# google/uis-rnn

Measured on NVIDIA H100. Metric: predict_frames_per_sec_beam10_256d, higher is better.
Workload: dtype f32

## Files before the change

### uisrnn_b200/csrc/uis_beam.cuh

```cuda
#pragma once
#include "uis_common.cuh"
#include "uis_beam_tc.cuh"
#include "uis_beam_stat.cuh"

namespace uis {

constexpr int kStages = 2;
constexpr int kStageBytes = 48 * 1024;
constexpr int kInitSlot = 0;
#ifndef UIS_CP_BEAM
#define UIS_CP_BEAM 20
#endif
constexpr int kCPBeam = UIS_CP_BEAM;
template <int H> struct BeamCP { static constexpr int value = H > 512 ? 8 : kCPBeam; };
template <int H> __host__ __device__ constexpr int beam_cp() { return BeamCP<H>::value; }
constexpr int kCPCluster = 12;
constexpr int kXchVals = 24;
constexpr int kCPTree = 16;
template <int H> struct TreeCP { static constexpr int value = H > 512 ? 8 : kCPTree; };
template <int H> __host__ __device__ constexpr int tree_cp() { return TreeCP<H>::value; }
constexpr int kMaxLanes = 8;
constexpr int kMaxBeam = 128;
constexpr int kMaxDepth = 4;

// ... 37 lines not shown
  alignas(64) CUtensorMap tc_wmap;
  float tc_sh, tc_sa;
  float tc_inv_hh, tc_inv_1, tc_inv_2;
  float* tc_scratch;
  SmemLayout tc_layout;
  unsigned* stat_bar;
  float* stat_scratch;
  float* pool_mean;
  float* pool_hidden;
  float* pool_mse;
  unsigned* bp;
  int* queue;
  int* labels;
  int* status;
  unsigned long long* stats;
  int trace_utt;
  int trace_capacity;
  int* dbg_win;
  float* dbg_score;
  long long* dbg_off;
  float* dbg_final_scores;
  int* dbg_final_k;
  float* dbg_best_mean;
  float* dbg_best_hidden;
  int* dbg_best_blocks;
  unsigned char* tree_arena;
  int tree_spill_all;
};

template <int V> struct Pow2Floor { static constexpr int value = (V >= 2) ? 2 * Pow2Floor<V / 2>::value : 1; };
template <> struct Pow2Floor<1> { static constexpr int value = 1; };
template <> struct Pow2Floor<0> { static constexpr int value = 1; };
constexpr int cmin(int a, int b) { return a < b ? a : b; }

template <int H_, int D_, int CP_ = kCPBeam>
struct Cfg {
  static constexpr int H = H_, D = D_;
  static constexpr int CP = CP_;
  static constexpr int UPT = (H >= 512) ? 2 : 1;
  static constexpr int NT = H / UPT;
  static constexpr int NW = NT / 32;
  static constexpr bool REBALANCE = (NT == 256);
  static constexpr int PRODUCER_THREADS = REBALANCE ? 128 : 32;
  static constexpr int BLOCK = NT + PRODUCER_THREADS;
  static constexpr int RG = 3 * UPT;
  static constexpr int KG1 = UPT, TG1 = NT / KG1, R1 = H / TG1;
  static constexpr int R2 = (UPT == 2) ? 4 : 1, KG2 = NT * R2 / D, TG2 = NT / KG2;
  static constexpr int KT_HH = Pow2Floor<kStageBytes / (12 * H)>::value;
  static constexpr int KT_1 = cmin(Pow2Floor<kStageBytes / (4 * H)>::value, H);
  static constexpr int KT_2 = cmin(Pow2Floor<kStageBytes / (4 * D)>::value, H);
  static constexpr int N_HH = H / KT_HH, N_1 = H / KT_1, N_2 = H / KT_2;
  static constexpr int TILES_PER_PASS = N_HH + N_1 + N_2;
  static_assert(H % KT_HH == 0 && H % KT_1 == 0 && H % KT_2 == 0, "tile split");
  static_assert(KT_1 % KG1 == 0 && KT_2 % KG2 == 0, "K split");
  static_assert(TG2 * R2 == D && TG1 * R1 == H, "row split");
  static_assert(KG1 * H <= 2 * H && KG2 * D <= 2 * H, "K-split scratch must fit in XA+XB");
  static_assert(D % 4 == 0 && NT % 32 == 0 && D <= NT, "shape");
};

__host__ __device__ inline unsigned align_up(unsigned v, unsigned a) { return (v + a - 1) / a * a; }

enum { LS_U = 0, LS_N, LS_TN, LS_T, LS_NB, LS_GEN, LS_ACTIVE, LS_FAILED, LS_TRACED, LS_NFINITE, LS_KMAX,
       LS_NWIN, LS_ERR, LS_M, LS_COLBASE, LS_NE, LS_ROW0_LO, LS_ROW0_HI, LS_DBGROWS_LO, LS_DBGROWS_HI,
       LS_FRESH, LS_COUNT = 24 };
enum { MI_PUBLISHED = 0, MI_DONE, MI_MTOT, MI_QNEXT, MI_NLIST, MI_MAXK };

template <int H, int D, int kCP = kCPBeam, bool XCL = false, int TCN = 0, bool STAT = false>
__host__ __device__ inline SmemLayout make_layout(int B, int Kcap, int G) {
  SmemLayout L;
  unsigned o = 0;
  if constexpr (TCN > 0) {
    using TC = TcCfg<H, D, TCN>;
    L.ring = o;  o += TC::STAGES * kTcBoxBytes;
    L.xa = o;    o += TC::BOP_BYTES;
    L.xb = o;
  } else {
    L.ring = o;  o += STAT ? align_up(StatCfg<H, D>::BYTES, 128) : kStages * kStageBytes;
    L.xa = o;    o += H * kCP * 4;
    L.xb = o;    o += H * kCP * 4;
  }
  L.wv = o;    o += D * 4;
  unsigned q = 0;
  L.l_xt = q;      q += 2 * D * 4;
  L.l_tabs = q;    q += 2u * B * Kcap * 16;
  L.l_meta = q;    q += 2u * 4 * B * 4;
  L.l_candoff = q; q += align_up((B + 1) * 4, 16);
  const unsigned ne = (unsigned)B * (Kcap + 1);
  L.l_keys = q;    q += align_up(ne * 8, 16);
  L.l_svals = q;   q += align_up(ne * 4, 16);
  L.l_wins = q;    q += align_up(3u * B * 4, 16);
  L.l_wcol = q;    q += align_up((unsigned)B * 4, 16);
  L.l_lcol = q;    q += align_up(2u * B * 4, 16);
  const unsigned pw = ((unsigned)B * Kcap + B + 1 + 31) / 32;
  L.l_used = q;    q += align_up(pw * 4, 16);
  L.l_scored = q;  q += align_up(pw * 4, 16);
  L.l_ls = q;      q += LS_COUNT * 4;
  L.lane_stride = align_up(q, 16);
  L.lanes = o;     o += L.lane_stride * G;
// ... 465 lines not shown
    const int m = i / H, k = i % H;
    XA[(size_t)k * CP + m] = __ldcg(pool_hidden_g + (size_t)cc.lane[m0 + m] * lane_pool_h + (size_t)cc.dst[m0 + m] * H + k);
  }
  named_bar_sync(1, NT);
  stat_dot<H, S::R1, CP, NT>(sW, S::LD, S::R0, XA, XB, Mp, tid);
  named_bar_sync(1, NT);
  if (tid < S::R1 * CP) {
    const int m = tid % CP, u = tid / CP, j = q * S::R1 + u;
    if (m < Mp)
      scratch_g[(size_t)m * H + j] = fmaxf(__fadd_rn(stat_sum<S::R1, CP, NT>(XB, u, m), __ldg(p.b1 + j)), 0.f);
  }
  stat_group_sync<NT>(bar, epoch, tid);
  if (tid == 0) { const long long now_ = clock64(); ph[3] += now_ - tmark; tmark = now_; }
  for (int i = tid; i < Mp * H; i += NT) {
    const int m = i / H, k = i % H;
    XA[(size_t)k * CP + m] = __ldcg(scratch_g + (size_t)m * H + k);
  }
  named_bar_sync(1, NT);
  stat_dot<H, S::R2, CP, NT>(sW, S::LD, S::R0 + S::R1, XA, XB, Mp, tid);
  named_bar_sync(1, NT);
  if (tid < S::R2 * CP) {
    const int m = tid % CP, u = tid / CP, d = q * S::R2 + u;
    if (m < Mp) {
      const float mval = __fadd_rn(stat_sum<S::R2, CP, NT>(XB, u, m), __ldg(p.b2 + d));
      const int n = cc.vis[m0 + m];
      const float mu_old = __ldcg(pool_mean_g + (size_t)cc.lane[m0 + m] * lane_pool_m + (size_t)cc.src[m0 + m] * D + d);
      const float mu = (n == 0) ? mval : __fdiv_rn(__fadd_rn(__fmul_rn(mu_old, (float)(n - 1)), mval), (float)n);
      pool_mean_g[(size_t)cc.lane[m0 + m] * lane_pool_m + (size_t)cc.dst[m0 + m] * D + d] = mu;
    }
  }
  stat_group_sync<NT>(bar, epoch, tid);
}

template <int H, int D, int N, class Idle>
__device__ __forceinline__ void tc_run_pass(const BeamParams& p, const unsigned char* ring, unsigned char* bop,
                                            const TcBars& tb, unsigned& tbox, const ColCtx cc, int m0, int Mp,
                                            float* pool_mean_cta, float* pool_hidden_cta, float* scratch_cta, int tid,
                                            int lane, int warp, long long* ph, long long& tmark, long long* tstat,
                                            Idle idle_work) {
  using TC = TcCfg<H, D, N>;
  constexpr int NT = 256, NI = N / 8;
  constexpr int KB = (NI == 6) ? 2 : 4, WB = (NI == 6) ? 3 : NI;
  auto hslot = [&](int g, int s) { return pool_hidden_cta + (size_t)(g * p.P + s) * H; };
  auto mslot = [&](int g, int s) { return pool_mean_cta + (size_t)(g * p.P + s) * D; };
  const int wg = warp >> 2;
  const int r0 = wg * 64 + (warp & 3) * 16 + (lane >> 2);
  const int cq = 2 * (lane & 3);
  long long* ts = (tid == 0) ? tstat : nullptr;
  const long long t_in = clock64();
  float acc[TC::NACC];
  auto stage_b = [&](auto src, float scale) {
    const long long w0 = clock64();
    tc_gather_b<H, N, NT>(bop, src, Mp, scale, tid);
    tc_publish_b<NT>();
    if (ts) ts[2] += clock64() - w0;
  };
  if (tid < Mp && (tid == 0 || cc.lane[m0 + tid] != cc.lane[m0 + tid - 1]))
    prefetch_l2_bulk(p.gi + (size_t)cc.girow[m0 + tid] * 3 * H, 3 * H * 4);
  stage_b([&](int m) -> const float* {
    return hslot(cc.lane[m0 + m], cc.src[m0 + m]); }, p.tc_sh);
  if (tid == 0) { const long long now_ = clock64(); ph[1] += now_ - tmark; tmark = now_; }
  idle_work();
  if (tid == 0) { const long long now_ = clock64(); ph[7] += now_ - tmark; tmark = now_; }
  static_assert(H >= NT, "gate parking: 2 * (N / 2) * NT floats within the [N][H] scratch");
  float* park = scratch_cta + tid;
  for (int ut = 0; ut < TC::UT; ++ut) {
    const int j0 = ut * 128 + r0;
    {
      float v[TC::NV];
#pragma unroll
      for (int g = 0; g < 2; ++g) {
        tc_tile<TC>(acc, ring, bop, tb, tbox, wg, lane, ts);
        tc_fold<TC>(acc, v, p.tc_inv_hh);
        const float bh[2] = {__ldg(p.bhh + g * H + j0), __ldg(p.bhh + g * H + j0 + 8)};
#pragma unroll
        for (int q = 0; q < TC::NV; ++q) park[(g * TC::NV + q) * NT] = __fadd_rn(v[q], bh[(q >> 1) & 1]);
      }
    }
    tc_tile<TC>(acc, ring, bop, tb, tbox, wg, lane, ts);
    float an[TC::NV];
    tc_fold<TC>(acc, an, p.tc_inv_hh);
    {
      const float bh[2] = {__ldg(p.bhh + 2 * H + j0), __ldg(p.bhh + 2 * H + j0 + 8)};
#pragma unroll
      for (int q = 0; q < TC::NV; ++q) an[q] = __fadd_rn(an[q], bh[(q >> 1) & 1]);
    }
#pragma unroll
    for (int k0 = 0; k0 < 2 * NI; k0 += KB) {
      float gr[KB][2], gz[KB][2], gn[KB][2], pr[KB][2], pz[KB][2], ho[KB][2];
#pragma unroll
      for (int b = 0; b < KB; ++b) {
        const int i = (k0 + b) >> 1, e = (k0 + b) & 1, m = 8 * i + cq + e;
        if (m < Mp) {
          const float* gi = p.gi + (size_t)cc.girow[m0 + m] * 3 * H + j0;
          const float* hs = hslot(cc.lane[m0 + m], cc.src[m0 + m]) + j0;
#pragma unroll
// ... 109 lines not shown
  uint64_t* empty = full + (TC ? TCC::STAGES : kStages);
  volatile int* misc = reinterpret_cast<volatile int*>(smem + L.misc);
  TcBars tb{full, empty};

  const int tid = threadIdx.x, lane = tid & 31, warp = tid >> 5;

  if (tid == 0) {
    if constexpr (TC) {
      for (int s = 0; s < TCC::STAGES; ++s) {
        mbar_init(&tb.full[s], 1);
        mbar_init(&tb.empty[s], NW);
      }
    } else {
      for (int s = 0; s < kStages; ++s) {
        mbar_init(&full[s], 1);
        mbar_init(&empty[s], NW);
      }
    }
    for (int i = 0; i < 16; ++i) misc[i] = 0;
    if constexpr (TC)
      for (int i = 16; i < 20; ++i) reinterpret_cast<long long*>(smem + L.phase)[i] = 0;
    if constexpr (XCL) {
      uint64_t* xbar = reinterpret_cast<uint64_t*>(smem + L.xbar);
      mbar_init(&xbar[0], cluster_nctarank() - 1);
      mbar_init(&xbar[1], cluster_nctarank() - 1);
      misc[MI_QNEXT] = (int)cluster_id_x();
    }
    if constexpr (STAT) misc[MI_QNEXT] = sgroup;
    fence_mbar_init();
  }
  __syncthreads();
  if constexpr (XCL) cluster_sync_all();

  if (warp >= NW) {
    if constexpr (STAT) return;
    if constexpr (TC) asm volatile("setmaxnreg.dec.sync.aligned.u32 40;");
    else if constexpr (C::REBALANCE) asm volatile("setmaxnreg.dec.sync.aligned.u32 24;");
    if constexpr (TC) {
      if (warp == NW) tc_producer_loop<TCC, H>(&p.tc_wmap, reinterpret_cast<unsigned char*>(ring), tb, &misc[MI_DONE]);
    } else {
      if (warp == NW && lane == 0) producer_loop<C, XCL>(p, ring, full, empty, misc);
    }
    return;
  }
  if constexpr (TC) asm volatile("setmaxnreg.inc.sync.aligned.u32 232;");
  else if constexpr (C::REBALANCE && !STAT) asm volatile("setmaxnreg.inc.sync.aligned.u32 240;");

  auto lane_base = [&](int g) -> unsigned char* { return smem + L.lanes + (size_t)g * L.lane_stride; };
  auto LSp = [&](int g) -> volatile int* { return reinterpret_cast<volatile int*>(lane_base(g) + L.l_ls); };
  const int DH = p.depth * H;
  const size_t pool_m_stride = (size_t)p.P * D, pool_h_stride = (size_t)p.P * DH;
  float* pool_mean_cta = p.pool_mean + (size_t)(STAT ? sgroup : blockIdx.x) * G * pool_m_stride;
  float* pool_hidden_cta = p.pool_hidden + (size_t)(STAT ? sgroup : blockIdx.x) * G * pool_h_stride;
  unsigned* bp_cta = p.bp + (size_t)blockIdx.x * G * p.maxN * B;
  const unsigned PW = (unsigned)(p.P + 31) / 32;
  const float INF = __int_as_float(0x7f800000);
  const int bbits = B > 32 ? 7 : 5;

  float bh[C::RG], b1r[UPT];
#pragma unroll
  for (int i = 0; i < C::RG; ++i) bh[i] = TC ? 0.f : p.bhh[(i / UPT) * H + tid + NT * (i % UPT)];
#pragma unroll
  for (int u = 0; u < UPT; ++u) b1r[u] = TC ? 0.f : p.b1[tid + NT * u];
  const float b2r = (tid < D && !TC) ? p.b2[tid] : 0.f;
  unsigned tc_boxes = 0;
  float* tc_scratch_cta = TC ? p.tc_scratch + (size_t)blockIdx.x * (TC ? TCN : 1) * H : nullptr;
  if (tid < D) wv[tid] = p.wvec[tid];
  unsigned stat_epoch = 0;
  if constexpr (STAT) stat_load_weights<H, D, NT>(ring, p.whh_t, p.w1_t, p.w2_t, sq, tid);
  for (int g = 0; g < G; ++g) {
    if (tid < D) pool_mean_cta[g * pool_m_stride + (size_t)kInitSlot * D + tid] = p.mean0[tid];
    for (int q = tid; q < DH; q += NT) pool_hidden_cta[g * pool_h_stride + (size_t)kInitSlot * DH + q] = p.hidden0[q];
  }

  int* collane = colarr; int* colsrc = colarr + G * B; int* colnew = colarr + 2 * G * B;
  int* colvis = colarr + 3 * G * B;
  long long* colrow = reinterpret_cast<long long*>(colarr + 4 * G * B);
  const ColCtx cc{collane, colsrc, colnew, colvis, colrow};
  XchCtx xc{reinterpret_cast<float*>(smem + L.xch), reinterpret_cast<uint64_t*>(smem + L.xbar),
            XCL ? cluster_ctarank() : 0u, XCL ? cluster_nctarank() : 1u, 0u};
  const int xsize = (int)xc.size;

  unsigned it = 0;
  long long* ph = reinterpret_cast<long long*>(smem + L.phase);
  if (tid == 0) {
    for (int i = 0; i < 16; ++i) ph[i] = 0;
    ph[10] = clock64();
  }
  long long& tmark = ph[10];
  long long& st_cols = ph[11]; long long& st_pass = ph[12]; long long& st_cand = ph[13]; long long& st_steps = ph[14];
  long long& st_maxk = ph[15];
#define UIS_PHASE(i)                         \
  do {                                       \
    if (tid == 0) {                          \
      const long long now_ = clock64();      \
      ph[i] += now_ - tmark;                 \
      tmark = now_;                          \
    }                                        \
  } while (0)

  auto lane_fetch = [&](int g) {
    volatile int* ls = LSp(g);
    for (;;) {
      int uidx;
      if constexpr (XCL) {
        uidx = misc[MI_QNEXT];
        misc[MI_QNEXT] = uidx + (int)cluster_nclusters_x();
      } else if constexpr (STAT) {
        uidx = misc[MI_QNEXT];
        misc[MI_QNEXT] = uidx + (int)(gridDim.x / kStatGroup);
      } else {
        uidx = atomicAdd(p.queue, 1);
      }
      if (uidx >= p.U) { ls[LS_ACTIVE] = 0; ls[LS_FRESH] = 0; return; }
      const int u = p.order[uidx];
      const long long row0 = p.row_off[u];
      const int N = (int)(p.row_off[u + 1] - row0);
      if (N == 0) {
        p.status[u] = 0;
        if (p.dbg_final_scores) {
          for (int b = 0; b < B; ++b) p.dbg_final_scores[(size_t)u * B + b] = INF;
          if (p.dbg_final_k) p.dbg_final_k[u] = 0;
        }
        continue;
      }
      ls[LS_U] = u; ls[LS_N] = N; ls[LS_TN] = p.T * N; ls[LS_T] = 0; ls[LS_NB] = 1; ls[LS_GEN] = 0;
      ls[LS_ACTIVE] = 1; ls[LS_FAILED] = 0; ls[LS_TRACED] = (u == p.trace_utt); ls[LS_ERR] = 0;
      ls[LS_ROW0_LO] = (int)(row0 & 0xffffffffll); ls[LS_ROW0_HI] = (int)(row0 >> 32);
      ls[LS_DBGROWS_LO] = 0; ls[LS_DBGROWS_HI] = 0; ls[LS_FRESH] = 1;
      for (unsigned w = 0; w < PW; ++w) reinterpret_cast<unsigned*>(lane_base(g) + L.l_scored)[w] = 0;
      int* meta = reinterpret_cast<int*>(lane_base(g) + L.l_meta);
      meta[0] = 0; meta[B] = -1; meta[2 * B] = 0; reinterpret_cast<float*>(meta)[3 * B] = 0.f;
      if (u == p.trace_utt && p.dbg_off) p.dbg_off[0] = 0;
      return;
    }
  };
  auto lane_prefetch = [&](int g, int t) {
    volatile int* ls = LSp(g);
    const long long row0 = ((long long)ls[LS_ROW0_HI] << 32) | (unsigned)ls[LS_ROW0_LO];
    const long long r = row0 + (t % ls[LS_N]);
    float* xts = reinterpret_cast<float*>(lane_base(g) + L.l_xt) + (t & 1) * D;
    for (int q = tid; q < D / 4; q += NT) cp_async16(xts + q * 4, p.x + (size_t)r * D + q * 4);
  };

  float* pool_mse_cta = p.pool_mse + (size_t)blockIdx.x * G * p.P;
  unsigned* slist = reinterpret_cast<unsigned*>(smem + L.slist);
  const int slist_cap = 64 * G;
  auto score_live_slots = [&](bool next) {
    for (;;) {
      if (tid == 0) misc[MI_NLIST] = 0;
      named_bar_sync(1, NT);
      for (int f = tid; f < G * (int)PW; f += NT) {
        const int g = f / (int)PW, w = f % (int)PW;
        unsigned* used = reinterpret_cast<unsigned*>(lane_base(g) + L.l_used);
        unsigned* scored = reinterpret_cast<unsigned*>(lane_base(g) + L.l_scored);
        unsigned bits = next ? (scored[w] & ~used[w]) : (used[w] & ~scored[w]);
        if (!LSp(g)[LS_ACTIVE]) bits = 0;
        const int n = __popc(bits);
        if (n) {
          int pos = atomicAdd((int*)&misc[MI_NLIST], n);
          unsigned done = 0;
          while (bits && pos < slist_cap) {
            const int bit = __ffs(bits) - 1;
            bits &= bits - 1;
            done |= 1u << bit;
            slist[pos++] = ((unsigned)g << 16) | (unsigned)(w * 32 + bit);
          }
          if (next) used[w] |= done; else scored[w] |= done;
        }
      }
      named_bar_sync(1, NT);
      const int ntot = misc[MI_NLIST], nlist = min(ntot, slist_cap);
      constexpr int kBatch = 4;
      for (int f0 = warp * kBatch; f0 < nlist; f0 += NW * kBatch) {
        int cg[kBatch];
        unsigned cslot[kBatch];
        float4 m4[kBatch][(D + 127) / 128];
#pragma unroll
        for (int q = 0; q < kBatch; ++q) {
          const int f = f0 + q;
          cg[q] = -1; cslot[q] = 0;
          if (f < nlist) {
            const unsigned ent = slist[f];
            cg[q] = (int)(ent >> 16); cslot[q] = ent & 0xffffu;
            const float* mu = pool_mean_cta + cg[q] * pool_m_stride + (size_t)cslot[q] * D;
#pragma unroll
            for (int i = 0; i < (D + 127) / 128; ++i)
              if (lane * 4 + i * 128 < D)
                m4[q][i] = STAT ? __ldcg(reinterpret_cast<const float4*>(mu + lane * 4 + i * 128))
                                : *reinterpret_cast<const float4*>(mu + lane * 4 + i * 128);
          }
        }
        float acc[kBatch], d0sq[kBatch];
#pragma unroll
        for (int q = 0; q < kBatch; ++q) {
          acc[q] = 0.f; d0sq[q] = 1.f;
          const int g = cg[q] < 0 ? 0 : cg[q];
          const float* xs = reinterpret_cast<const float*>(lane_base(g) + L.l_xt) + ((LSp(g)[LS_T] + (next ? 1 : 0)) & 1) * D;
#pragma unroll
          for (int i = 0; i < (D + 127) / 128; ++i) {
            const int d = lane * 4 + i * 128;
            if (d < D && cg[q] >= 0) {
              const float4 x4 = *reinterpret_cast<const float4*>(xs + d);
              const float4 w4 = *reinterpret_cast<const float4*>(wv + d);
              const float e0 = __fsub_rn(m4[q][i].x, x4.x), e1 = __fsub_rn(m4[q][i].y, x4.y);
              const float e2 = __fsub_rn(m4[q][i].z, x4.z), e3 = __fsub_rn(m4[q][i].w, x4.w);
              const float q0 = __fmul_rn(e0, e0);
              if (d == 0) d0sq[q] = q0;
              acc[q] = __fadd_rn(acc[q], __fmul_rn(q0, w4.x));
              acc[q] = __fadd_rn(acc[q], __fmul_rn(__fmul_rn(e1, e1), w4.y));
              acc[q] = __fadd_rn(acc[q], __fmul_rn(__fmul_rn(e2, e2), w4.z));
              acc[q] = __fadd_rn(acc[q], __fmul_rn(__fmul_rn(e3, e3), w4.w));
            }
          }
        }
#pragma unroll
        for (int o = 16; o > 0; o >>= 1) {
#pragma unroll
          for (int q = 0; q < kBatch; ++q) acc[q] = __fadd_rn(acc[q], __shfl_xor_sync(0xffffffffu, acc[q], o));
        }
        float my_acc = acc[0], my_d0 = __shfl_sync(0xffffffffu, d0sq[0], 0);
        int my_g = cg[0];
        unsigned my_slot = cslot[0];
#pragma unroll
        for (int q = 1; q < kBatch; ++q) {
          const float dq = __shfl_sync(0xffffffffu, d0sq[q], 0);
          if (lane == q) { my_acc = acc[q]; my_d0 = dq; my_g = cg[q]; my_slot = cslot[q]; }
        }
        if (lane < kBatch && my_g >= 0) {
          if (my_d0 == 0.f) my_acc = __fdiv_rn(my_acc, 0.f);
          pool_mse_cta[(size_t)my_g * p.P + my_slot] = my_acc;
        }
      }
      named_bar_sync(1, NT);
      if (ntot <= slist_cap) break;
    }
  };

  if (tid < G) lane_fetch(tid);
  named_bar_sync(1, NT);
  for (int g = 0; g < G; ++g)
    if (LSp(g)[LS_ACTIVE]) lane_prefetch(g, 0);
  cp_async_commit();

  for (;;) {
    int nact = 0;
    for (int g = 0; g < G; ++g) nact += LSp(g)[LS_ACTIVE];
    if (nact == 0) break;

    if (tid == 0 && !TC) {
      __threadfence_block();
      misc[MI_PUBLISHED] = misc[MI_PUBLISHED] + 1;
    }
    if (tid < G) {
      const int g = tid;
      volatile int* ls = LSp(g);
      ls[LS_M] = 0; ls[LS_NWIN] = 0; ls[LS_NE] = 0;
      if (ls[LS_ACTIVE]) {
        const int* mK = reinterpret_cast<const int*>(lane_base(g) + L.l_meta) + ls[LS_GEN] * 4 * B;
        int* candoff = reinterpret_cast<int*>(lane_base(g) + L.l_candoff);
        int off = 0, kmax = 0;
        const int nb = ls[LS_NB];
        for (int b = 0; b < nb; ++b) { candoff[b] = off; off += mK[b] + 1; kmax = max(kmax, mK[b]); }
        candoff[nb] = off;
        ls[LS_NFINITE] = 0; ls[LS_KMAX] = kmax; ls[LS_NE] = off;
      }
    }
    for (int g = 0; g < G; ++g) {
      unsigned* used = reinterpret_cast<unsigned*>(lane_base(g) + L.l_used);
      unsigned* scored = reinterpret_cast<unsigned*>(lane_base(g) + L.l_scored);
      for (unsigned w = tid; w < PW; w += NT) {
        used[w] = (w == 0) ? 1u : 0u;
        if (!TC) scored[w] = 0;
      }
    }
    cp_async_wait_all();
    named_bar_sync(1, NT);
    UIS_PHASE(6);
    for (int g = 0; g < G; ++g) {
      volatile int* ls = LSp(g);
      if (ls[LS_ACTIVE] && ls[LS_T] + 1 < ls[LS_TN]) lane_prefetch(g, ls[LS_T] + 1);
    }
    cp_async_commit();

    {
      int ne_g[kMaxLanes], ne_tot = 0;
      for (int g = 0; g < G; ++g) { ne_g[g] = LSp(g)[LS_NE]; ne_tot += ne_g[g]; }
      for (int f = tid; f < ne_tot; f += NT) {
        int g = 0, e = f;
        while (e >= ne_g[g]) { e -= ne_g[g]; ++g; }
        volatile int* ls = LSp(g);
        const int gen = ls[LS_GEN];
        const int* mK = reinterpret_cast<const int*>(lane_base(g) + L.l_meta) + gen * 4 * B;
        const int* mLast = mK + B; const int* mTot = mK + 2 * B;
        const int* candoff = reinterpret_cast<const int*>(lane_base(g) + L.l_candoff);
        const TabEntry* tab = reinterpret_cast<const TabEntry*>(lane_base(g) + L.l_tabs) + (size_t)gen * B * Kcap;
        int b = 0;
        while (candoff[b + 1] <= e) ++b;
        const int c = e - candoff[b];
        int slot = kInitSlot;
        double pen;
        if (c < mK[b]) {
          const TabEntry en = tab[(size_t)b * Kcap + c];
          slot = en.slot;
          atomicOr(reinterpret_cast<unsigned*>(lane_base(g) + L.l_used) + (slot >> 5), 1u << (slot & 31));
          pen = (c == mLast[b]) ? p.log_1mp0 : (p.log_p0 + __ldg(p.logn + en.blocks)) - __ldg(p.logtot + mTot[b]);
        } else {
          pen = (p.log_p0 + p.log_alpha) - __ldg(p.logtot + mTot[b]);
        }
        reinterpret_cast<double*>(lane_base(g) + L.l_keys)[e] = pen;
        reinterpret_cast<unsigned*>(lane_base(g) + L.l_svals)[e] = (unsigned)slot | ((unsigned)b << 16) | ((unsigned)c << (16 + bbits));
      }
      named_bar_sync(1, NT);
      score_live_slots(false);
      for (int f = tid; f < ne_tot; f += NT) {
        int g = 0, e = f;
        while (e >= ne_g[g]) { e -= ne_g[g]; ++g; }
        volatile int* ls = LSp(g);
        const unsigned info = reinterpret_cast<const unsigned*>(lane_base(g) + L.l_svals)[e];
        const int b = (int)((info >> 16) & ((1u << bbits) - 1u)), c = (int)(info >> (16 + bbits));
        const float mse = pool_mse_cta[(size_t)g * p.P + (info & 0xffffu)];
        const float* mNl = reinterpret_cast<const float*>(lane_base(g) + L.l_meta) + ls[LS_GEN] * 4 * B + 3 * B;
        const double pen = reinterpret_cast<const double*>(lane_base(g) + L.l_keys)[e];
        const float loss = __double2float_rn((double)mse - pen);
        const float S = __fadd_rn(mNl[b], loss);
        reinterpret_cast<float*>(lane_base(g) + L.l_svals)[e] = S;
        const unsigned flat = (unsigned)(b * (ls[LS_KMAX] + 1) + c);
        reinterpret_cast<unsigned long long*>(lane_base(g) + L.l_keys)[e] =
            ((unsigned long long)float_order_key(S) << 32) | flat;
        if (S < INF) atomicAdd((int*)&ls[LS_NFINITE], 1);
      }
      named_bar_sync(1, NT);
      UIS_PHASE(7);

      for (int f = tid; f < ne_tot; f += NT) {
        int g = 0, e = f;
        while (e >= ne_g[g]) { e -= ne_g[g]; ++g; }
        volatile int* ls = LSp(g);
        const int nwin = min((int)ls[LS_NFINITE], B);
        const unsigned long long* keys = reinterpret_cast<const unsigned long long*>(lane_base(g) + L.l_keys);
        const unsigned long long k = keys[e];
        int rank = 0;
        for (int q = 0; q < ne_g[g]; ++q) rank += (keys[q] < k) ? 1 : 0;
        if (rank < nwin) {
          const int* candoff = reinterpret_cast<const int*>(lane_base(g) + L.l_candoff);
          int b = 0;
          while (candoff[b + 1] <= e) ++b;
// ... 171 lines not shown
          if (r == 0 && p.dbg_off) p.dbg_off[t + 1] = rows + nwin;
        }
      }
    }
    for (int f = tid; f < Mtot; f += NT) {
      int g = 0;
      while (g + 1 < G && f >= colbase[g + 1]) ++g;
      const int lc = f - colbase[g];
      const int* lcolsrc = reinterpret_cast<const int*>(lane_base(g) + L.l_lcol);
      collane[f] = g;
      colsrc[f] = lcolsrc[lc];
      colnew[f] = lcolsrc[B + lc];
      {
        volatile int* lsg = LSp(g);
        const long long row0g = ((long long)lsg[LS_ROW0_HI] << 32) | (unsigned)lsg[LS_ROW0_LO];
        colrow[f] = row0g + (lsg[LS_T] % lsg[LS_N]);
      }
    }
    constexpr int kColsPerPass = TC ? TCN : C::CP;
    const int npass = TC ? (Mtot + kColsPerPass - 1) / kColsPerPass : max(1, (Mtot + C::CP - 1) / C::CP);
    if (tid == 0) {
      for (int g = 0; g < G; ++g) {
        volatile int* ls = LSp(g);
        if (ls[LS_ACTIVE]) { st_cand += ls[LS_NE]; st_steps += 1; }
      }
      st_cols += Mtot;
      st_pass += npass;
      if (npass > 1 && !TC) { __threadfence_block(); misc[MI_PUBLISHED] = misc[MI_PUBLISHED] + (npass - 1); }
    }
    named_bar_sync(1, NT);

    UIS_PHASE(0);
    if constexpr (TC) {
      auto prescore = [&]() {
        cp_async_wait_all();
        for (int f = tid; f < G * (int)PW; f += NT) {
          const int g = f / (int)PW, w = f % (int)PW;
          reinterpret_cast<unsigned*>(lane_base(g) + L.l_used)[w] = 0;
          reinterpret_cast<unsigned*>(lane_base(g) + L.l_scored)[w] = 0;
        }
        named_bar_sync(1, NT);
        for (int f = tid; f < G * B * Kcap; f += NT) {
          const int g = f / (B * Kcap), r = (f / Kcap) % B, c = f % Kcap;
          volatile int* ls = LSp(g);
          const bool go_on = ls[LS_ACTIVE] && !ls[LS_ERR] && ls[LS_NWIN] > 0 && ls[LS_T] + 1 < ls[LS_TN];
          if (!go_on || r >= ls[LS_NWIN]) continue;
          const int ngen = ls[LS_GEN] ^ 1;
          const int* nK = reinterpret_cast<const int*>(lane_base(g) + L.l_meta) + ngen * 4 * B;
          unsigned* scored = reinterpret_cast<unsigned*>(lane_base(g) + L.l_scored);
          if (r == 0 && c == 0) atomicOr(scored, 1u);
          if (c < nK[r]) {
            const int slot = (reinterpret_cast<const TabEntry*>(lane_base(g) + L.l_tabs) + (size_t)ngen * B * Kcap)[(size_t)r * Kcap + c].slot;
            atomicOr(scored + (slot >> 5), 1u << (slot & 31));
          }
        }
        named_bar_sync(1, NT);
        for (int f = tid; f < Mtot; f += NT) {
          unsigned* scored = reinterpret_cast<unsigned*>(lane_base(collane[f]) + L.l_scored);
          atomicAnd(scored + (colnew[f] >> 5), ~(1u << (colnew[f] & 31)));
        }
        score_live_slots(true);
      };
      auto nothing = []() {};
      if (Mtot == 0)
        for (int f = tid; f < G * (int)PW; f += NT)
          reinterpret_cast<unsigned*>(lane_base(f / (int)PW) + L.l_scored)[f % (int)PW] = 0;
      for (int m0 = 0; m0 < Mtot; m0 += TCN) {
        if (m0 == 0)
          tc_run_pass<H, D, TC ? TCN : 16>(p, reinterpret_cast<const unsigned char*>(ring), reinterpret_cast<unsigned char*>(XA),
                                           tb, tc_boxes, cc, m0, min(TCN, Mtot - m0), pool_mean_cta, pool_hidden_cta,
                                           tc_scratch_cta, tid, lane, warp, ph, tmark, ph + 16, prescore);
        else
          tc_run_pass<H, D, TC ? TCN : 16>(p, reinterpret_cast<const unsigned char*>(ring), reinterpret_cast<unsigned char*>(XA),
                                           tb, tc_boxes, cc, m0, min(TCN, Mtot - m0), pool_mean_cta, pool_hidden_cta,
                                           tc_scratch_cta, tid, lane, warp, ph, tmark, ph + 16, nothing);
        named_bar_sync(1, NT);
        UIS_PHASE(4);
      }
    } else {
    if (Mtot == 0 && !STAT) drain_pass<C>(full, empty, it, lane, p.depth, xsize);
    for (int m0 = 0; m0 < Mtot; m0 += C::CP) {
      const int Mp = min(C::CP, Mtot - m0);
#pragma unroll
      for (int u = 0; u < UPT; ++u) {
        const int j = tid + NT * u;
#pragma unroll
        for (int c = 0; c < C::CP / 4; ++c) {
          float hv[4];
#pragma unroll
          for (int q = 0; q < 4; ++q) {
            const int m = 4 * c + q;
            const float* hp = pool_hidden_cta + (size_t)collane[m0 + m] * pool_h_stride + (size_t)colsrc[m0 + m] * DH + j;
            hv[q] = (m < Mp) ? (STAT ? __ldcg(hp) : *hp) : 0.f;
          }
          reinterpret_cast<float4*>(XA + (size_t)j * C::CP)[c] = make_float4(hv[0], hv[1], hv[2], hv[3]);
        }
      }
      named_bar_sync(1, NT);
      UIS_PHASE(1);
      if constexpr (STAT)
        stat_pass<H, D, C::CP, NT>(p, ring, XA, XB, cc, m0, Mp, pool_mean_cta, pool_hidden_cta,
                                   p.stat_scratch + (size_t)sgroup * C::CP * H, p.stat_bar + (size_t)sgroup * kStatGroup, stat_epoch, sq, tid, ph, tmark);
      else if (p.dbg_mode == 1) drain_pass<C>(full, empty, it, lane, p.depth, xsize);
      else run_pass_any<C, DEEP, XCL>(p, ring, full, empty, it, XA, XB, cc, m0, Mp, pool_mean_cta, pool_hidden_cta, bh, b1r, b2r, tid, lane, ph, tmark, &xc);
      named_bar_sync(1, NT);
      UIS_PHASE(4);
    }
    }

    int fin[kMaxLanes];
    for (int g = 0; g < G; ++g) {
// ... 18 lines not shown
        for (int c = 0; c < fK[0]; ++c) {
          const TabEntry en = ftab[c];
          if (tid < D) p.dbg_best_mean[(size_t)c * D + tid] = pool_mean_cta[g * pool_m_stride + (size_t)en.slot * D + tid];
          for (int q = tid; q < DH; q += NT)
            p.dbg_best_hidden[(size_t)c * DH + q] = pool_hidden_cta[g * pool_h_stride + (size_t)en.slot * DH + q];
          if (tid == 0) p.dbg_best_blocks[c] = en.blocks;
        }
      }
    }
    named_bar_sync(1, NT);
    if (tid < G) {
      const int g = tid;
      volatile int* ls = LSp(g);
      if (ls[LS_ACTIVE]) {
        if (fin[g]) {
          const int u = ls[LS_U], N = ls[LS_N];
          const long long row0 = ((long long)ls[LS_ROW0_HI] << 32) | (unsigned)ls[LS_ROW0_LO];
          if (STAT && sq != 0) {
          } else if (ls[LS_ERR] || ls[LS_NWIN] == 0) {
            p.status[u] = ls[LS_ERR] ? -4 : -1;
            for (int i = 0; i < N; ++i) p.labels[row0 + i] = -1;
          } else {
            p.status[u] = 0;
            const unsigned* bp = bp_cta + (size_t)g * p.maxN * B;
            int r = 0;
            for (int i = N - 1; i >= 0; --i) {
              const unsigned e = bp[(size_t)i * B + r];
              p.labels[row0 + i] = (int)(e & 0xffffu);
              r = (int)(e >> 16);
            }
          }
          lane_fetch(g);
        } else {
          const long long rows = (((long long)ls[LS_DBGROWS_HI] << 32) | (unsigned)ls[LS_DBGROWS_LO]) + ls[LS_NWIN];
          ls[LS_DBGROWS_LO] = (int)(rows & 0xffffffffll); ls[LS_DBGROWS_HI] = (int)(rows >> 32);
          ls[LS_T] = ls[LS_T] + 1; ls[LS_NB] = ls[LS_NWIN]; ls[LS_GEN] = ls[LS_GEN] ^ 1; ls[LS_FRESH] = 0;
        }
      }
    }
    named_bar_sync(1, NT);
    {
      bool any = false;
      for (int g = 0; g < G; ++g)
        if (fin[g] && LSp(g)[LS_ACTIVE] && LSp(g)[LS_FRESH]) { lane_prefetch(g, 0); any = true; }
      if (any) cp_async_commit();
    }
    UIS_PHASE(5);
  }

  cp_async_wait_all();
  if constexpr (XCL) xch_barrier<NT>(xc, tid);
  if (tid == 0) {
    __threadfence_block();
    misc[MI_DONE] = 1;
    if (XCL && xc.rank != 0) return;
    if (STAT && sq != 0) return;
    atomicAdd(&p.stats[0], (unsigned long long)st_cols);
    atomicAdd(&p.stats[1], (unsigned long long)st_pass);
    atomicAdd(&p.stats[2], (unsigned long long)st_cand);
    atomicAdd(&p.stats[3], (unsigned long long)st_steps);
    atomicMax(&p.stats[4], (unsigned long long)max(st_maxk, (long long)misc[MI_MAXK]));
    for (int i = 0; i < 10; ++i) atomicAdd(&p.stats[8 + i], (unsigned long long)ph[i]);
    if constexpr (TC)
      for (int i = 0; i < 4; ++i) atomicAdd(&p.stats[18 + i], (unsigned long long)ph[16 + i]);
  }
}

}
```

### uisrnn_b200/csrc/uis_common.cuh

```cuda
#pragma once
#include <cuda_runtime.h>
#include <stdint.h>

namespace uis {

struct DeviceGuard {
  int prev = -1;
  cudaError_t status = cudaSuccess;
  explicit DeviceGuard(int device) {
    if (cudaGetDevice(&prev) != cudaSuccess) prev = -1;
    status = (prev == device) ? cudaSuccess : cudaSetDevice(device);
  }
  ~DeviceGuard() {
    int now = -1;
    if (prev >= 0 && cudaGetDevice(&now) == cudaSuccess && now != prev) cudaSetDevice(prev);
  }
  DeviceGuard(const DeviceGuard&) = delete;
  DeviceGuard& operator=(const DeviceGuard&) = delete;
};

__device__ __forceinline__ uint32_t smem_u32(const void* p) {
  return static_cast<uint32_t>(__cvta_generic_to_shared(p));
}

// ... 98 lines not shown
        : "r"(smem_u32(bar)), "r"(parity)
        : "memory");
  } while (!ok);
}
__device__ __forceinline__ void cluster_sync_all() {
  asm volatile("barrier.cluster.arrive.release.aligned;\n\tbarrier.cluster.wait.acquire.aligned;" ::: "memory");
}

__device__ __forceinline__ void tma_bulk_g2s(void* smem_dst, const void* gmem_src,
                                             uint32_t bytes, uint64_t* bar) {
  asm volatile(
      "cp.async.bulk.shared::cluster.global.mbarrier::complete_tx::bytes [%0], [%1], %2, [%3];" ::
          "r"(smem_u32(smem_dst)),
      "l"(gmem_src), "r"(bytes), "r"(smem_u32(bar))
      : "memory");
}

__device__ __forceinline__ void prefetch_l2_bulk(const void* gmem_src, uint32_t bytes) {
  asm volatile("cp.async.bulk.prefetch.L2.global [%0], %1;" ::"l"(gmem_src), "r"(bytes) : "memory");
}

__device__ __forceinline__ void cp_async16(void* smem_dst, const void* gmem_src) {
  asm volatile("cp.async.cg.shared.global [%0], [%1], 16;" ::"r"(smem_u32(smem_dst)),
               "l"(gmem_src)
               : "memory");
}
__device__ __forceinline__ void cp_async_commit() { asm volatile("cp.async.commit_group;" ::: "memory"); }
__device__ __forceinline__ void cp_async_wait_all() { asm volatile("cp.async.wait_group 0;" ::: "memory"); }
__device__ __forceinline__ void cp_async_wait_but_one() { asm volatile("cp.async.wait_group 1;" ::: "memory"); }

__device__ __forceinline__ void named_bar_sync(int id, int nthreads) {
  asm volatile("bar.sync %0, %1;" ::"r"(id), "r"(nthreads) : "memory");
}

__device__ __forceinline__ float warp_sum(float v) {
#pragma unroll
  for (int o = 16; o > 0; o >>= 1) v += __shfl_xor_sync(0xffffffffu, v, o);
  return v;
}

__device__ __forceinline__ uint32_t float_order_key(float f) {
  if (f != f) return 0xffffffffu;
  uint32_t u = __float_as_uint(f);
  return (u & 0x80000000u) ? ~u : (u | 0x80000000u);
}

__device__ __forceinline__ float float_from_order_key(uint32_t k) {
  return __uint_as_float((k & 0x80000000u) ? (k & 0x7fffffffu) : ~k);
}

__device__ __forceinline__ float sigmoid_f32(float v) {
  return __fdiv_rn(1.0f, __fadd_rn(1.0f, expf(-v)));
}

}
```

Before: 2.062 million.

## Offload prescore and next-step prelude to helper warps during tensor-core passes

In the tensor-core path, the previously idle extra warps (beyond the producer warp) become 96 helper threads. A handshake over named barriers drives them. While the consumer warps run the tensor-core GEMM passes, the helpers prefetch the next frame, rebuild the used/scored bitmaps, score live slots, and, when no lane finishes, advance lane state and compute the next step's candidate penalties, so the main loop can skip those phases. This moves serial bookkeeping off the critical path. The cost is more complex synchronisation, epoch checks that trap on mismatch, and helpers limited to 40 registers.

```diff
diff --git a/uisrnn_b200/csrc/uis_beam.cuh b/uisrnn_b200/csrc/uis_beam.cuh
--- a/uisrnn_b200/csrc/uis_beam.cuh
+++ b/uisrnn_b200/csrc/uis_beam.cuh
@@ -93,6 +93,7 @@
 template <> struct Pow2Floor<1> { static constexpr int value = 1; };
 template <> struct Pow2Floor<0> { static constexpr int value = 1; };
 constexpr int cmin(int a, int b) { return a < b ? a : b; }
+template <int V> struct IntConst { static constexpr int value = V; };
 
 template <int H_, int D_, int CP_ = kCPBeam>
 struct Cfg {
@@ -124,7 +125,12 @@
 enum { LS_U = 0, LS_N, LS_TN, LS_T, LS_NB, LS_GEN, LS_ACTIVE, LS_FAILED, LS_TRACED, LS_NFINITE, LS_KMAX,
        LS_NWIN, LS_ERR, LS_M, LS_COLBASE, LS_NE, LS_ROW0_LO, LS_ROW0_HI, LS_DBGROWS_LO, LS_DBGROWS_HI,
        LS_FRESH, LS_COUNT = 24 };
-enum { MI_PUBLISHED = 0, MI_DONE, MI_MTOT, MI_QNEXT, MI_NLIST, MI_MAXK };
+enum { MI_PUBLISHED = 0, MI_DONE, MI_MTOT, MI_QNEXT, MI_NLIST, MI_MAXK, MI_HMODE, MI_HEPOCH, MI_HACK };
+enum { HELP_PRELUDE = 0,
+       HELP_PRESCORE = 1,
+       HELP_EXIT = 2 };
+constexpr int kBarHandA = 2, kBarHandB = 3, kBarHelpers = 4;
+constexpr int kHelperThreads = 96;
 
 template <int H, int D, int kCP = kCPBeam, bool XCL = false, int TCN = 0, bool STAT = false>
 __host__ __device__ inline SmemLayout make_layout(int B, int Kcap, int G) {
@@ -656,12 +662,11 @@
   stat_group_sync<NT>(bar, epoch, tid);
 }
 
-template <int H, int D, int N, class Idle>
+template <int H, int D, int N>
 __device__ __forceinline__ void tc_run_pass(const BeamParams& p, const unsigned char* ring, unsigned char* bop,
                                             const TcBars& tb, unsigned& tbox, const ColCtx cc, int m0, int Mp,
                                             float* pool_mean_cta, float* pool_hidden_cta, float* scratch_cta, int tid,
-                                            int lane, int warp, long long* ph, long long& tmark, long long* tstat,
-                                            Idle idle_work) {
+                                            int lane, int warp, long long* ph, long long& tmark, long long* tstat) {
   using TC = TcCfg<H, D, N>;
   constexpr int NT = 256, NI = N / 8;
   constexpr int KB = (NI == 6) ? 2 : 4, WB = (NI == 6) ? 3 : NI;
@@ -684,8 +689,6 @@
   stage_b([&](int m) -> const float* {
     return hslot(cc.lane[m0 + m], cc.src[m0 + m]); }, p.tc_sh);
   if (tid == 0) { const long long now_ = clock64(); ph[1] += now_ - tmark; tmark = now_; }
-  idle_work();
-  if (tid == 0) { const long long now_ = clock64(); ph[7] += now_ - tmark; tmark = now_; }
   static_assert(H >= NT, "gate parking: 2 * (N / 2) * NT floats within the [N][H] scratch");
   float* park = scratch_cta + tid;
   for (int ut = 0; ut < TC::UT; ++ut) {
@@ -861,19 +864,13 @@
   __syncthreads();
   if constexpr (XCL) cluster_sync_all();
 
-  if (warp >= NW) {
+  if (warp >= NW && !TC) {
     if constexpr (STAT) return;
-    if constexpr (TC) asm volatile("setmaxnreg.dec.sync.aligned.u32 40;");
-    else if constexpr (C::REBALANCE) asm volatile("setmaxnreg.dec.sync.aligned.u32 24;");
-    if constexpr (TC) {
-      if (warp == NW) tc_producer_loop<TCC, H>(&p.tc_wmap, reinterpret_cast<unsigned char*>(ring), tb, &misc[MI_DONE]);
-    } else {
-      if (warp == NW && lane == 0) producer_loop<C, XCL>(p, ring, full, empty, misc);
-    }
+    if constexpr (C::REBALANCE) asm volatile("setmaxnreg.dec.sync.aligned.u32 24;");
+    if (warp == NW && lane == 0) producer_loop<C, XCL>(p, ring, full, empty, misc);
     return;
   }
-  if constexpr (TC) asm volatile("setmaxnreg.inc.sync.aligned.u32 232;");
-  else if constexpr (C::REBALANCE && !STAT) asm volatile("setmaxnreg.inc.sync.aligned.u32 240;");
+  if constexpr (C::REBALANCE && !STAT && !TC) asm volatile("setmaxnreg.inc.sync.aligned.u32 240;");
 
   auto lane_base = [&](int g) -> unsigned char* { return smem + L.lanes + (size_t)g * L.lane_stride; };
   auto LSp = [&](int g) -> volatile int* { return reinterpret_cast<volatile int*>(lane_base(g) + L.l_ls); };
@@ -897,7 +894,7 @@
   if (tid < D) wv[tid] = p.wvec[tid];
   unsigned stat_epoch = 0;
   if constexpr (STAT) stat_load_weights<H, D, NT>(ring, p.whh_t, p.w1_t, p.w2_t, sq, tid);
-  for (int g = 0; g < G; ++g) {
+  for (int g = 0; g < G && warp < NW; ++g) {
     if (tid < D) pool_mean_cta[g * pool_m_stride + (size_t)kInitSlot * D + tid] = p.mean0[tid];
     for (int q = tid; q < DH; q += NT) pool_hidden_cta[g * pool_h_stride + (size_t)kInitSlot * DH + q] = p.hidden0[q];
   }
@@ -964,22 +961,28 @@
       return;
     }
   };
-  auto lane_prefetch = [&](int g, int t) {
+  auto lane_prefetch = [&](int g, int t, int me, int nthr) {
     volatile int* ls = LSp(g);
     const long long row0 = ((long long)ls[LS_ROW0_HI] << 32) | (unsigned)ls[LS_ROW0_LO];
     const long long r = row0 + (t % ls[LS_N]);
     float* xts = reinterpret_cast<float*>(lane_base(g) + L.l_xt) + (t & 1) * D;
-    for (int q = tid; q < D / 4; q += NT) cp_async16(xts + q * 4, p.x + (size_t)r * D + q * 4);
+    for (int q = me; q < D / 4; q += nthr) cp_async16(xts + q * 4, p.x + (size_t)r * D + q * 4);
+  };
+  auto lane_advance = [&](int g) {
+    volatile int* ls = LSp(g);
+    const long long rows = (((long long)ls[LS_DBGROWS_HI] << 32) | (unsigned)ls[LS_DBGROWS_LO]) + ls[LS_NWIN];
+    ls[LS_DBGROWS_LO] = (int)(rows & 0xffffffffll); ls[LS_DBGROWS_HI] = (int)(rows >> 32);
+    ls[LS_T] = ls[LS_T] + 1; ls[LS_NB] = ls[LS_NWIN]; ls[LS_GEN] = ls[LS_GEN] ^ 1; ls[LS_FRESH] = 0;
   };
 
   float* pool_mse_cta = p.pool_mse + (size_t)blockIdx.x * G * p.P;
   unsigned* slist = reinterpret_cast<unsigned*>(smem + L.slist);
   const int slist_cap = 64 * G;
-  auto score_live_slots = [&](bool next) {
+  auto score_live_slots = [&](bool next, int me, int nthr, int w0, int nw, int bar, auto batch) {
     for (;;) {
-      if (tid == 0) misc[MI_NLIST] = 0;
-      named_bar_sync(1, NT);
-      for (int f = tid; f < G * (int)PW; f += NT) {
+      if (me == 0) misc[MI_NLIST] = 0;
+      named_bar_sync(bar, nthr);
+      for (int f = me; f < G * (int)PW; f += nthr) {
         const int g = f / (int)PW, w = f % (int)PW;
         unsigned* used = reinterpret_cast<unsigned*>(lane_base(g) + L.l_used);
         unsigned* scored = reinterpret_cast<unsigned*>(lane_base(g) + L.l_scored);
@@ -998,10 +1001,10 @@
           if (next) used[w] |= done; else scored[w] |= done;
         }
       }
-      named_bar_sync(1, NT);
+      named_bar_sync(bar, nthr);
       const int ntot = misc[MI_NLIST], nlist = min(ntot, slist_cap);
-      constexpr int kBatch = 4;
-      for (int f0 = warp * kBatch; f0 < nlist; f0 += NW * kBatch) {
+      constexpr int kBatch = decltype(batch)::value;
+      for (int f0 = w0 * kBatch; f0 < nlist; f0 += nw * kBatch) {
         int cg[kBatch];
         unsigned cslot[kBatch];
         float4 m4[kBatch][(D + 127) / 128];
@@ -1061,28 +1064,14 @@
           pool_mse_cta[(size_t)my_g * p.P + my_slot] = my_acc;
         }
       }
-      named_bar_sync(1, NT);
+      named_bar_sync(bar, nthr);
       if (ntot <= slist_cap) break;
     }
   };
 
-  if (tid < G) lane_fetch(tid);
-  named_bar_sync(1, NT);
-  for (int g = 0; g < G; ++g)
-    if (LSp(g)[LS_ACTIVE]) lane_prefetch(g, 0);
-  cp_async_commit();
-
-  for (;;) {
-    int nact = 0;
-    for (int g = 0; g < G; ++g) nact += LSp(g)[LS_ACTIVE];
-    if (nact == 0) break;
-
-    if (tid == 0 && !TC) {
-      __threadfence_block();
-      misc[MI_PUBLISHED] = misc[MI_PUBLISHED] + 1;
-    }
-    if (tid < G) {
-      const int g = tid;
+  auto step_p0 = [&](int me, int nthr) {
+    if (me < G) {
+      const int g = me;
       volatile int* ls = LSp(g);
       ls[LS_M] = 0; ls[LS_NWIN] = 0; ls[LS_NE] = 0;
       if (ls[LS_ACTIVE]) {
@@ -1098,50 +1087,149 @@
     for (int g = 0; g < G; ++g) {
       unsigned* used = reinterpret_cast<unsigned*>(lane_base(g) + L.l_used);
       unsigned* scored = reinterpret_cast<unsigned*>(lane_base(g) + L.l_scored);
-      for (unsigned w = tid; w < PW; w += NT) {
+      for (unsigned w = me; w < PW; w += nthr) {
         used[w] = (w == 0) ? 1u : 0u;
         if (!TC) scored[w] = 0;
       }
     }
-    cp_async_wait_all();
-    named_bar_sync(1, NT);
-    UIS_PHASE(6);
-    for (int g = 0; g < G; ++g) {
+  };
+  auto step_p1a = [&](int me, int nthr, const int (&ne_g)[kMaxLanes], int ne_tot) {
+    for (int f = me; f < ne_tot; f += nthr) {
+      int g = 0, e = f;
+      while (e >= ne_g[g]) { e -= ne_g[g]; ++g; }
       volatile int* ls = LSp(g);
-      if (ls[LS_ACTIVE] && ls[LS_T] + 1 < ls[LS_TN]) lane_prefetch(g, ls[LS_T] + 1);
-    }
-    cp_async_commit();
+      const int gen = ls[LS_GEN];
+      const int* mK = reinterpret_cast<const int*>(lane_base(g) + L.l_meta) + gen * 4 * B;
+      const int* mLast = mK + B; const int* mTot = mK + 2 * B;
+      const int* candoff = reinterpret_cast<const int*>(lane_base(g) + L.l_candoff);
+      const TabEntry* tab = reinterpret_cast<const TabEntry*>(lane_base(g) + L.l_tabs) + (size_t)gen * B * Kcap;
+      int b = 0;
+      while (candoff[b + 1] <= e) ++b;
+      const int c = e - candoff[b];
+      int slot = kInitSlot;
+      double pen;
+      if (c < mK[b]) {
+        const TabEntry en = tab[(size_t)b * Kcap + c];
+        slot = en.slot;
+        atomicOr(reinterpret_cast<unsigned*>(lane_base(g) + L.l_used) + (slot >> 5), 1u << (slot & 31));
+        pen = (c == mLast[b]) ? p.log_1mp0 : (p.log_p0 + __ldg(p.logn + en.blocks)) - __ldg(p.logtot + mTot[b]);
+      } else {
+        pen = (p.log_p0 + p.log_alpha) - __ldg(p.logtot + mTot[b]);
+      }
+      reinterpret_cast<double*>(lane_base(g) + L.l_keys)[e] = pen;
+      reinterpret_cast<unsigned*>(lane_base(g) + L.l_svals)[e] = (unsigned)slot | ((unsigned)b << 16) | ((unsigned)c << (16 + bbits));
+    }
+  };
+
+  if constexpr (TC) {
+    if (warp < NW) {
+      asm volatile("setmaxnreg.inc.sync.aligned.u32 232;");
+    } else {
+      asm volatile("setmaxnreg.dec.sync.aligned.u32 40;");
+      if (warp == NW) {
+        tc_producer_loop<TCC, H>(&p.tc_wmap, reinterpret_cast<unsigned char*>(ring), tb, &misc[MI_DONE]);
+        return;
+      }
+      const int me = tid - NT - 32, hwarp = warp - NW - 1;
+      constexpr int HT = kHelperThreads;
+      for (int epoch = 1;; ++epoch) {
+        named_bar_sync(kBarHandA, NT + HT);
+        if (misc[MI_HEPOCH] != epoch) __trap();
+        const int mode = misc[MI_HMODE];
+        if (mode == HELP_EXIT) return;
+        auto go_on = [&](int g) {
+          volatile int* ls = LSp(g);
+          return ls[LS_ACTIVE] && !ls[LS_ERR] && ls[LS_NWIN] > 0 && ls[LS_T] + 1 < ls[LS_TN];
+        };
+        for (int g = 0; g < G; ++g)
+          if (go_on(g)) lane_prefetch(g, LSp(g)[LS_T] + 1, me, HT);
+        cp_async_commit();
+        for (int f = me; f < G * (int)PW; f += HT) {
+          const int g = f / (int)PW, w = f % (int)PW;
+          reinterpret_cast<unsigned*>(lane_base(g) + L.l_used)[w] = 0;
+          reinterpret_cast<unsigned*>(lane_base(g) + L.l_scored)[w] = 0;
+        }
+        cp_async_wait_all();
+        named_bar_sync(kBarHelpers, HT);
+        for (int f = me; f < G * B * Kcap; f += HT) {
+          const int g = f / (B * Kcap), r = (f / Kcap) % B, c = f % Kcap;
+          volatile int* ls = LSp(g);
+          if (!go_on(g) || r >= ls[LS_NWIN]) continue;
+          const int ngen = ls[LS_GEN] ^ 1;
+          const int* nK = reinterpret_cast<const int*>(lane_base(g) + L.l_meta) + ngen * 4 * B;
+          unsigned* scored = reinterpret_cast<unsigned*>(lane_base(g) + L.l_scored);
+          if (r == 0 && c == 0) atomicOr(scored, 1u);
+          if (c < nK[r]) {
+            const int slot = (reinterpret_cast<const TabEntry*>(lane_base(g) + L.l_tabs) + (size_t)ngen * B * Kcap)[(size_t)r * Kcap + c].slot;
+            atomicOr(scored + (slot >> 5), 1u << (slot & 31));
+          }
+        }
+        named_bar_sync(kBarHelpers, HT);
+        const int Mtot = misc[MI_MTOT];
+        for (int f = me; f < Mtot; f += HT) {
+          unsigned* scored = reinterpret_cast<unsigned*>(lane_base(collane[f]) + L.l_scored);
+          atomicAnd(scored + (colnew[f] >> 5), ~(1u << (colnew[f] & 31)));
+        }
+        score_live_slots(true, me, HT, hwarp, HT / 32, kBarHelpers, IntConst<1>{});
+        if (mode == HELP_PRELUDE) {
+          if (me < G && LSp(me)[LS_ACTIVE]) lane_advance(me);
+          named_bar_sync(kBarHelpers, HT);
+          step_p0(me, HT);
+          named_bar_sync(kBarHelpers, HT);
+          int ne_g[kMaxLanes], ne_tot = 0;
+          for (int g = 0; g < G; ++g) { ne_g[g] = LSp(g)[LS_NE]; ne_tot += ne_g[g]; }
+          step_p1a(me, HT, ne_g, ne_tot);
+        }
+        if (me == 0) misc[MI_HACK] = epoch;
+        named_bar_arrive(kBarHandB, NT + HT);
+      }
+    }
+  }
+
+  if (tid < G) lane_fetch(tid);
+  named_bar_sync(1, NT);
+  for (int g = 0; g < G; ++g)
+    if (LSp(g)[LS_ACTIVE]) lane_prefetch(g, 0, tid, NT);
+  cp_async_commit();
+
+  bool helped = false;
+  for (;;) {
+    if (!helped) {
+      int nact = 0;
+      for (int g = 0; g < G; ++g) nact += LSp(g)[LS_ACTIVE];
+      if (nact == 0) {
+        if constexpr (TC) {
+          if (tid == 0) { misc[MI_HMODE] = HELP_EXIT; misc[MI_HEPOCH] = misc[MI_HEPOCH] + 1; }
+          named_bar_arrive(kBarHandA, NT + kHelperThreads);
+        }
+        break;
+      }
+
+      if (tid == 0 && !TC) {
+        __threadfence_block();
+        misc[MI_PUBLISHED] = misc[MI_PUBLISHED] + 1;
+      }
+      step_p0(tid, NT);
+      cp_async_wait_all();
+      named_bar_sync(1, NT);
+      UIS_PHASE(6);
+      if constexpr (!TC) {
+        for (int g = 0; g < G; ++g) {
+          volatile int* ls = LSp(g);
+          if (ls[LS_ACTIVE] && ls[LS_T] + 1 < ls[LS_TN]) lane_prefetch(g, ls[LS_T] + 1, tid, NT);
+        }
+        cp_async_commit();
+      }
+    }
 
     {
       int ne_g[kMaxLanes], ne_tot = 0;
       for (int g = 0; g < G; ++g) { ne_g[g] = LSp(g)[LS_NE]; ne_tot += ne_g[g]; }
-      for (int f = tid; f < ne_tot; f += NT) {
-        int g = 0, e = f;
-        while (e >= ne_g[g]) { e -= ne_g[g]; ++g; }
-        volatile int* ls = LSp(g);
-        const int gen = ls[LS_GEN];
-        const int* mK = reinterpret_cast<const int*>(lane_base(g) + L.l_meta) + gen * 4 * B;
-        const int* mLast = mK + B; const int* mTot = mK + 2 * B;
-        const int* candoff = reinterpret_cast<const int*>(lane_base(g) + L.l_candoff);
-        const TabEntry* tab = reinterpret_cast<const TabEntry*>(lane_base(g) + L.l_tabs) + (size_t)gen * B * Kcap;
-        int b = 0;
-        while (candoff[b + 1] <= e) ++b;
-        const int c = e - candoff[b];
-        int slot = kInitSlot;
-        double pen;
-        if (c < mK[b]) {
-          const TabEntry en = tab[(size_t)b * Kcap + c];
-          slot = en.slot;
-          atomicOr(reinterpret_cast<unsigned*>(lane_base(g) + L.l_used) + (slot >> 5), 1u << (slot & 31));
-          pen = (c == mLast[b]) ? p.log_1mp0 : (p.log_p0 + __ldg(p.logn + en.blocks)) - __ldg(p.logtot + mTot[b]);
-        } else {
-          pen = (p.log_p0 + p.log_alpha) - __ldg(p.logtot + mTot[b]);
-        }
-        reinterpret_cast<double*>(lane_base(g) + L.l_keys)[e] = pen;
-        reinterpret_cast<unsigned*>(lane_base(g) + L.l_svals)[e] = (unsigned)slot | ((unsigned)b << 16) | ((unsigned)c << (16 + bbits));
-      }
-      named_bar_sync(1, NT);
-      score_live_slots(false);
+      if (!helped) {
+        step_p1a(tid, NT, ne_g, ne_tot);
+        named_bar_sync(1, NT);
+      }
+      score_live_slots(false, tid, NT, warp, NW, 1, IntConst<4>{});
       for (int f = tid; f < ne_tot; f += NT) {
         int g = 0, e = f;
         while (e >= ne_g[g]) { e -= ne_g[g]; ++g; }
@@ -1379,51 +1467,29 @@
 
     UIS_PHASE(0);
     if constexpr (TC) {
-      auto prescore = [&]() {
-        cp_async_wait_all();
-        for (int f = tid; f < G * (int)PW; f += NT) {
-          const int g = f / (int)PW, w = f % (int)PW;
-          reinterpret_cast<unsigned*>(lane_base(g) + L.l_used)[w] = 0;
-          reinterpret_cast<unsigned*>(lane_base(g) + L.l_scored)[w] = 0;
-        }
-        named_bar_sync(1, NT);
-        for (int f = tid; f < G * B * Kcap; f += NT) {
-          const int g = f / (B * Kcap), r = (f / Kcap) % B, c = f % Kcap;
+      if (tid == 0) {
+        bool anyfin = false;
+        for (int g = 0; g < G; ++g) {
           volatile int* ls = LSp(g);
-          const bool go_on = ls[LS_ACTIVE] && !ls[LS_ERR] && ls[LS_NWIN] > 0 && ls[LS_T] + 1 < ls[LS_TN];
-          if (!go_on || r >= ls[LS_NWIN]) continue;
-          const int ngen = ls[LS_GEN] ^ 1;
-          const int* nK = reinterpret_cast<const int*>(lane_base(g) + L.l_meta) + ngen * 4 * B;
-          unsigned* scored = reinterpret_cast<unsigned*>(lane_base(g) + L.l_scored);
-          if (r == 0 && c == 0) atomicOr(scored, 1u);
-          if (c < nK[r]) {
-            const int slot = (reinterpret_cast<const TabEntry*>(lane_base(g) + L.l_tabs) + (size_t)ngen * B * Kcap)[(size_t)r * Kcap + c].slot;
-            atomicOr(scored + (slot >> 5), 1u << (slot & 31));
-          }
-        }
-        named_bar_sync(1, NT);
-        for (int f = tid; f < Mtot; f += NT) {
-          unsigned* scored = reinterpret_cast<unsigned*>(lane_base(collane[f]) + L.l_scored);
-          atomicAnd(scored + (colnew[f] >> 5), ~(1u << (colnew[f] & 31)));
-        }
-        score_live_slots(true);
-      };
-      auto nothing = []() {};
-      if (Mtot == 0)
-        for (int f = tid; f < G * (int)PW; f += NT)
-          reinterpret_cast<unsigned*>(lane_base(f / (int)PW) + L.l_scored)[f % (int)PW] = 0;
+          anyfin |= ls[LS_ACTIVE] && (ls[LS_ERR] || ls[LS_NWIN] == 0 || ls[LS_T] + 1 >= ls[LS_TN]);
+        }
+        misc[MI_MTOT] = Mtot;
+        misc[MI_HMODE] = anyfin ? HELP_PRESCORE : HELP_PRELUDE;
+        misc[MI_HEPOCH] = misc[MI_HEPOCH] + 1;
+      }
+      named_bar_arrive(kBarHandA, NT + kHelperThreads);
       for (int m0 = 0; m0 < Mtot; m0 += TCN) {
-        if (m0 == 0)
-          tc_run_pass<H, D, TC ? TCN : 16>(p, reinterpret_cast<const unsigned char*>(ring), reinterpret_cast<unsigned char*>(XA),
-                                           tb, tc_boxes, cc, m0, min(TCN, Mtot - m0), pool_mean_cta, pool_hidden_cta,
-                                           tc_scratch_cta, tid, lane, warp, ph, tmark, ph + 16, prescore);
-        else
-          tc_run_pass<H, D, TC ? TCN : 16>(p, reinterpret_cast<const unsigned char*>(ring), reinterpret_cast<unsigned char*>(XA),
-                                           tb, tc_boxes, cc, m0, min(TCN, Mtot - m0), pool_mean_cta, pool_hidden_cta,
-                                           tc_scratch_cta, tid, lane, warp, ph, tmark, ph + 16, nothing);
+        tc_run_pass<H, D, TC ? TCN : 16>(p, reinterpret_cast<const unsigned char*>(ring), reinterpret_cast<unsigned char*>(XA),
+                                         tb, tc_boxes, cc, m0, min(TCN, Mtot - m0), pool_mean_cta, pool_hidden_cta,
+                                         tc_scratch_cta, tid, lane, warp, ph, tmark, ph + 16);
         named_bar_sync(1, NT);
         UIS_PHASE(4);
       }
+      named_bar_sync(kBarHandB, NT + kHelperThreads);
+      if (tid == 0 && misc[MI_HACK] != misc[MI_HEPOCH]) __trap();
+      UIS_PHASE(6);
+      helped = misc[MI_HMODE] == HELP_PRELUDE;
+      if (helped) continue;
     } else {
     if (Mtot == 0 && !STAT) drain_pass<C>(full, empty, it, lane, p.depth, xsize);
     for (int m0 = 0; m0 < Mtot; m0 += C::CP) {
@@ -1508,9 +1574,7 @@
           }
           lane_fetch(g);
         } else {
-          const long long rows = (((long long)ls[LS_DBGROWS_HI] << 32) | (unsigned)ls[LS_DBGROWS_LO]) + ls[LS_NWIN];
-          ls[LS_DBGROWS_LO] = (int)(rows & 0xffffffffll); ls[LS_DBGROWS_HI] = (int)(rows >> 32);
-          ls[LS_T] = ls[LS_T] + 1; ls[LS_NB] = ls[LS_NWIN]; ls[LS_GEN] = ls[LS_GEN] ^ 1; ls[LS_FRESH] = 0;
+          lane_advance(g);
         }
       }
     }
@@ -1518,7 +1582,7 @@
     {
       bool any = false;
       for (int g = 0; g < G; ++g)
-        if (fin[g] && LSp(g)[LS_ACTIVE] && LSp(g)[LS_FRESH]) { lane_prefetch(g, 0); any = true; }
+        if (fin[g] && LSp(g)[LS_ACTIVE] && LSp(g)[LS_FRESH]) { lane_prefetch(g, 0, tid, NT); any = true; }
       if (any) cp_async_commit();
     }
     UIS_PHASE(5);
diff --git a/uisrnn_b200/csrc/uis_common.cuh b/uisrnn_b200/csrc/uis_common.cuh
--- a/uisrnn_b200/csrc/uis_common.cuh
+++ b/uisrnn_b200/csrc/uis_common.cuh
@@ -154,6 +154,9 @@
 __device__ __forceinline__ void named_bar_sync(int id, int nthreads) {
   asm volatile("bar.sync %0, %1;" ::"r"(id), "r"(nthreads) : "memory");
 }
+__device__ __forceinline__ void named_bar_arrive(int id, int nthreads) {
+  asm volatile("bar.arrive %0, %1;" ::"r"(id), "r"(nthreads) : "memory");
+}
 
 __device__ __forceinline__ float warp_sum(float v) {
 #pragma unroll
```

Measured after the change: 2.268 million (median of 6 runs). 1.1x the previous value.
